# zeromq/libzmq

Hardware: AMD Instinct MI355X
Metric: GiB/s device-resident CURVE encode+decode, 1 KiB-msg batches; msgs/s (higher is better)
Workload: dtype u32; 1 GPU; config2: 65536 x 1024 B frames, 1 CURVE session per GPU, encode+decode round trip; frames_per_gpu=65536, payload_bytes=1024, wire_bytes=1057, sessions=1, parallelism=frame-sharded x1, no collective

## Files before the change

### libzmq_amd/csrc/curve_device.hpp

```cpp
#pragma once

#include <hip/hip_runtime.h>
#include <stdint.h>

namespace zmqg {

__device__ __forceinline__ uint32_t rotl32(uint32_t x, uint32_t n)
{
    return __builtin_rotateleft32(x, n);
}

#define ZMQG_QR(a, b, c, d)        \
    b ^= rotl32(a + d, 7);         \
    c ^= rotl32(b + a, 9);         \
    d ^= rotl32(c + b, 13);        \
    a ^= rotl32(d + c, 18);

#define ZMQG_SALSA20_ROUNDS(x)                                   \
    _Pragma("unroll") for (int rr_ = 0; rr_ < 10; ++rr_)         \
    {                                                            \
        ZMQG_QR(x[0], x[4], x[8], x[12]);                        \
        ZMQG_QR(x[5], x[9], x[13], x[1]);                        \
        ZMQG_QR(x[10], x[14], x[2], x[6]);                       \
        ZMQG_QR(x[15], x[3], x[7], x[11]);                       \
// ... 355 lines not shown
        a = poly32_add(h, c[8], c[9], c[10], c[11], 1u);
    } else {
        a = poly32_add(h, c[0], c[1], c[2], c[3], 1u);
        a = poly32_mul_add<true>(a, k, c[4], c[5], c[6], c[7], 1u);
        a = poly32_mul_add<true>(a, k, c[8], c[9], c[10], c[11], 1u);
    }
    a = poly32_mul_add<true>(a, k, c[12], c[13], c[14], c[15], 1u);
    h = poly32_mul_add<false>(a, k, 0u, 0u, 0u, 0u, 0u);
}

__device__ __forceinline__ PolyKey32 poly32_key_from_fe(const uint32_t r[5])
{
    return poly32_key(r[0] | (r[1] << 26), (r[1] >> 6) | (r[2] << 20), (r[2] >> 12) | (r[3] << 14),
                      (r[3] >> 18) | (r[4] << 8));
}

__device__ __forceinline__ Poly32 fe_to_poly32(fe x)
{
    uint32_t c;
    c = x.l[0] >> 26;
    x.l[0] &= M26;
    x.l[1] += c;
    c = x.l[1] >> 26;
    x.l[1] &= M26;
    x.l[2] += c;
    c = x.l[2] >> 26;
    x.l[2] &= M26;
    x.l[3] += c;
    c = x.l[3] >> 26;
    x.l[3] &= M26;
    x.l[4] += c;
    Poly32 h;
    h.h0 = x.l[0] | (x.l[1] << 26);
    h.h1 = (x.l[1] >> 6) | (x.l[2] << 20);
    h.h2 = (x.l[2] >> 12) | (x.l[3] << 14);
    h.h3 = (x.l[3] >> 18) | (x.l[4] << 8);
    h.h4 = x.l[4] >> 24;
    return h;
}

__device__ __forceinline__ fe poly32_to_fe(const Poly32 &h)
{
    fe x;
    x.l[0] = h.h0 & M26;
    x.l[1] = ((h.h0 >> 26) | (h.h1 << 6)) & M26;
    x.l[2] = ((h.h1 >> 20) | (h.h2 << 12)) & M26;
    x.l[3] = ((h.h2 >> 14) | (h.h3 << 18)) & M26;
    x.l[4] = (h.h3 >> 8) | (h.h4 << 24);
    return x;
}

__device__ __forceinline__ void poly32_finish(const Poly32 &h, const uint32_t s[4], uint32_t tag[4])
{
    unsigned c;
    const uint32_t g0 = __builtin_addc(h.h0, 5u, 0u, &c);
    const uint32_t g1 = __builtin_addc(h.h1, 0u, c, &c);
    const uint32_t g2 = __builtin_addc(h.h2, 0u, c, &c);
    const uint32_t g3 = __builtin_addc(h.h3, 0u, c, &c);
    const uint32_t g4 = h.h4 + c;
    const uint32_t m = 0u - (g4 >> 2);
    const uint32_t f0 = (g0 & m) | (h.h0 & ~m), f1 = (g1 & m) | (h.h1 & ~m), f2 = (g2 & m) | (h.h2 & ~m),
                   f3 = (g3 & m) | (h.h3 & ~m);
    tag[0] = __builtin_addc(f0, s[0], 0u, &c);
    tag[1] = __builtin_addc(f1, s[1], c, &c);
    tag[2] = __builtin_addc(f2, s[2], c, &c);
    tag[3] = __builtin_addc(f3, s[3], c, &c);
}

__device__ __forceinline__ uint32_t bswap32(uint32_t x)
{
    return __builtin_bswap32(x);
}

__device__ __forceinline__ void mask_tail(uint32_t w[16], int nv)
{
#pragma unroll
    for (int i = 0; i < 16; ++i) {
        const int b = nv - 4 * i;
        const uint32_t m = b >= 4 ? 0xffffffffu : (b <= 0 ? 0u : ((1u << (8 * b)) - 1u));
        w[i] &= m;
    }
}

__device__ __forceinline__ void load_window(const uint8_t *p, int nv, uint32_t w[16])
{
    const uint32_t sh = (uint32_t) ((uintptr_t) p & 3);
    const uint32_t *q = (const uint32_t *) (p - sh);
    uint32_t d[17];
    if (nv >= 64) {
#pragma unroll
        for (int i = 0; i < 16; ++i)
            d[i] = q[i];
        d[16] = sh ? q[16] : 0u;
    } else {
        const int nd = (int) ((sh + (uint32_t) nv + 3) >> 2);
#pragma unroll
        for (int i = 0; i < 17; ++i)
            d[i] = i < nd ? q[i] : 0u;
    }
#pragma unroll
    for (int i = 0; i < 16; ++i)
        w[i] = __builtin_amdgcn_alignbyte(d[i + 1], d[i], sh);
    if (nv < 64)
        mask_tail(w, nv);
}

__device__ __forceinline__ void store_window(uint8_t *p, int nv, const uint32_t w[16])
{
    const uintptr_t a = (uintptr_t) p;
    const uint32_t sh = (uint32_t) (a & 3);
    if (sh == 0 && nv >= 64) {
        typedef unsigned int u32x4_ __attribute__((ext_vector_type(4)));
        typedef __attribute__((address_space(1))) u32x4_ __attribute__((aligned(4))) GU4a4_;
#pragma unroll
        for (int i = 0; i < 4; ++i)
            *(GU4a4_ *) (a + 16u * i) = (u32x4_){w[4 * i], w[4 * i + 1], w[4 * i + 2], w[4 * i + 3]};
        return;
    }
    const uint32_t s = (4u - sh) & 3u;
    (void) a;
    uint32_t e[16];
#pragma unroll
    for (int k = 0; k < 15; ++k)
        e[k] = __builtin_amdgcn_alignbyte(w[k + 1], w[k], s);
    e[15] = __builtin_amdgcn_alignbyte(0u, w[15], s);
    const int lead = (int) s < nv ? (int) s : nv;
#pragma unroll
    for (int b = 0; b < 3; ++b)
        if (b < lead)
            p[b] = (uint8_t) (w[0] >> (8 * b));
    if (nv <= (int) s)
        return;
    const int rem = nv - (int) s;
    const int nd = rem >> 2;
    uint32_t *q = (uint32_t *) (p + s);
#pragma unroll
    for (int k = 0; k < 16; ++k)
        if (k < nd)
            q[k] = e[k];
    const int tb = rem & 3;
    if (tb) {
        uint32_t t = 0;
#pragma unroll
        for (int k = 0; k < 16; ++k)
            if (k == nd)
                t = e[k];
        uint8_t *pt = (uint8_t *) (q + nd);
#pragma unroll
        for (int b = 0; b < 3; ++b)
            if (b < tb)
                pt[b] = (uint8_t) (t >> (8 * b));
    }
}

template <int NV>
__device__ __forceinline__ void store_bytes_c(uint8_t *p, const uint32_t w[16])
{
    static_assert(NV % 4 == 0 && NV >= 8 && NV <= 64, "whole dwords, at most one window");
    typedef __attribute__((address_space(1))) uint8_t GU8_;
    typedef __attribute__((address_space(1))) uint16_t GU16_;
    typedef __attribute__((address_space(1))) uint32_t GU32_;
    typedef unsigned int u32x2_ __attribute__((ext_vector_type(2)));
    typedef unsigned int u32x3_ __attribute__((ext_vector_type(3)));
    typedef __attribute__((address_space(1))) u32x2_ __attribute__((aligned(4))) GU2a4_;
    typedef __attribute__((address_space(1))) u32x3_ __attribute__((aligned(4))) GU3a4_;
    typedef unsigned int u32x4_ __attribute__((ext_vector_type(4)));
    typedef __attribute__((address_space(1))) u32x4_ __attribute__((aligned(4))) GU4a4_;
    const uint64_t a = (uint64_t) (uintptr_t) p;
    const uint32_t sh = (uint32_t) a & 3u, s = (4u - sh) & 3u;
    constexpr int ND = NV / 4;
    uint32_t e[ND];
#pragma unroll
    for (int k = 0; k < ND; ++k)
        e[k] = __builtin_amdgcn_alignbyte(k + 1 < 16 ? w[k + 1] : 0u, w[k], s);
    if (s & 1u)
        *(GU8_ *) (uintptr_t) a = (uint8_t) w[0];
    if (s & 2u)
        *(GU16_ *) (uintptr_t) (a + (s & 1u)) = (uint16_t) (w[0] >> (8u * (s & 1u)));
    const uint64_t q = a + s;
    constexpr int NU = ND - 1;
#pragma unroll
    for (int g = 0; g + 4 <= NU; g += 4)
        *(GU4a4_ *) (uintptr_t) (q + 4u * g) = (u32x4_){e[g], e[g + 1], e[g + 2], e[g + 3]};
    constexpr int G4 = NU / 4 * 4;
    if (NU - G4 == 3)
        *(GU3a4_ *) (uintptr_t) (q + 4u * G4) = (u32x3_){e[G4], e[G4 + 1], e[G4 + 2]};
    else if (NU - G4 == 2)
        *(GU2a4_ *) (uintptr_t) (q + 4u * G4) = (u32x2_){e[G4], e[G4 + 1]};
    else if (NU - G4 == 1)
        *(GU32_ *) (uintptr_t) (q + 4u * G4) = e[G4];
    if (s == 0u)
        *(GU32_ *) (uintptr_t) (q + 4u * NU) = e[NU];
    const uint64_t t = q + 4u * NU;
    if (sh & 2u)
        *(GU16_ *) (uintptr_t) t = (uint16_t) e[NU];
    if (sh & 1u)
        *(GU8_ *) (uintptr_t) (t + (sh & 2u)) = (uint8_t) (e[NU] >> (8u * (sh & 2u)));
}

template <int NV>
__device__ __forceinline__ void load_bytes_c(const uint8_t *p, uint32_t w[NV / 4])
{
    static_assert(NV % 16 == 0 && NV >= 16 && NV <= 48, "whole granules");
    typedef __attribute__((address_space(1))) const uint32_t GCU32_;
    typedef unsigned int u32x4_ __attribute__((ext_vector_type(4)));
    typedef __attribute__((address_space(1))) const u32x4_ __attribute__((aligned(4))) GCU4a4_;
    const uint64_t a = (uint64_t) (uintptr_t) p;
    const uint32_t sh = (uint32_t) a & 3u;
    const uint64_t q = a - sh;
    constexpr int ND = NV / 4;
    uint32_t d[ND + 1];
#pragma unroll
    for (int g = 0; g < ND / 4; ++g) {
        const u32x4_ t = *(GCU4a4_ *) (uintptr_t) (q + 16u * g);
        d[4 * g] = t.x;
        d[4 * g + 1] = t.y;
        d[4 * g + 2] = t.z;
        d[4 * g + 3] = t.w;
    }
    d[ND] = sh ? *(GCU32_ *) (uintptr_t) (q + 4u * ND) : 0u;
#pragma unroll
    for (int k = 0; k < ND; ++k)
        w[k] = __builtin_amdgcn_alignbyte(d[k + 1], d[k], sh);
}

__device__ __forceinline__ void store_tail(uint64_t a, uint32_t nb, const uint32_t o[17])
{
    typedef __attribute__((address_space(1))) uint8_t GU8_;
    typedef __attribute__((address_space(1))) uint16_t GU16_;
    typedef __attribute__((address_space(1))) uint32_t GU32_;
    typedef unsigned int u32x4_ __attribute__((ext_vector_type(4)));
    typedef __attribute__((address_space(1))) u32x4_ __attribute__((aligned(4))) GU4a4_;
    const uint32_t nw = nb >> 2, ng = nw >> 2;
#pragma unroll
    for (uint32_t g = 0; g < 4; ++g)
        if (g < ng)
            *(GU4a4_ *) (uintptr_t) (a + 16u * g) = (u32x4_){o[4 * g], o[4 * g + 1], o[4 * g + 2], o[4 * g + 3]};
    uint32_t r[4];
#pragma unroll
    for (uint32_t k = 0; k < 4; ++k) {
        uint32_t v = 0;
#pragma unroll
        for (uint32_t g = 0; g < 5; ++g)
            if (g == ng && 4 * g + k < 17)
                v = o[4 * g + k];
        r[k] = v;
    }
    const uint64_t b = a + 16u * ng;
    const uint32_t nr = nw - 4u * ng;
#pragma unroll
    for (uint32_t k = 0; k < 3; ++k)
        if (k < nr)
            *(GU32_ *) (uintptr_t) (b + 4u * k) = r[k];
    uint32_t last = r[0];
#pragma unroll
    for (uint32_t k = 1; k < 4; ++k)
        if (k == nr)
            last = r[k];
    const uint32_t tb = nb & 3u;
    const uint64_t c = b + 4u * nr;
    if (tb & 2u)
        *(GU16_ *) (uintptr_t) c = (uint16_t) last;
    if (tb & 1u)
        *(GU8_ *) (uintptr_t) (c + (tb & 2u)) = (uint8_t) (last >> (8u * (tb & 2u)));
}

__device__ __forceinline__ void zero_bytes(uint8_t *p, uint32_t len)
{
    const uint32_t head = (uint32_t) ((16u - ((uintptr_t) p & 15u)) & 15u);
    const uint32_t h = head < len ? head : len;
    for (uint32_t b = 0; b < h; ++b)
        p[b] = 0;
    uint32_t k = h;
    typedef unsigned int z4 __attribute__((ext_vector_type(4)));
    for (; k + 16u <= len; k += 16u)
        *(z4 *) (p + k) = (z4){0u, 0u, 0u, 0u};
    for (; k < len; ++k)
        p[k] = 0;
}

typedef unsigned int u32x4 __attribute__((ext_vector_type(4)));
typedef __attribute__((address_space(1))) uint8_t GU8;
typedef __attribute__((address_space(1))) const u32x4 GCU4;
typedef __attribute__((address_space(1))) u32x4 GU4;
typedef __attribute__((address_space(1))) uint32_t GU32;

template <int N>
__device__ __forceinline__ void select_shift(const uint32_t *v, uint32_t ws, uint32_t *out)
{
    const uint32_t m1 = 0u - (ws & 1u), m2 = 0u - ((ws >> 1) & 1u);
    uint32_t a[N + 2];
#pragma unroll
    for (int i = 0; i < N + 2; ++i)
        a[i] = (v[i + 1] & m1) | (v[i] & ~m1);
#pragma unroll
    for (int i = 0; i < N; ++i)
        out[i] = (a[i + 2] & m2) | (a[i] & ~m2);
}

struct StreamReader {
    const GCU4 *g;
    uint32_t off;
    uint32_t end;
// ... 163 lines not shown
```

### libzmq_amd/csrc/curve_frames.hpp

```cpp
#pragma once

#include "../../include/zmqg_curve.h"
#include "curve_device.hpp"
#include "curve_lbrec.hpp"
#include <type_traits>

namespace zmqg {

constexpr uint32_t kFramesBS = 256, kFramesWaves = kFramesBS / 64;

__device__ __forceinline__ void seq_store4(uint64_t a, uint32_t x, uint32_t y, uint32_t z, uint32_t w)
{
    typedef unsigned int v4_ __attribute__((ext_vector_type(4)));
    typedef __attribute__((address_space(1))) v4_ __attribute__((aligned(4))) G4_;
    *(G4_ *) (uintptr_t) a = (v4_){x, y, z, w};
}

#ifndef ZMQG_SEQ_STAMPS
#define ZMQG_SEQ_STAMPS 0
#endif

#if ZMQG_SEQ_STAMPS
#define SEQ_STAMP(slot)                                                                            \
    do {                                                                                           \
// ... 308 lines not shown
        __hip_atomic_store(&zs->done, 0u, __ATOMIC_RELAXED, __HIP_MEMORY_SCOPE_AGENT);
        __hip_atomic_store(&zs->ticket, 0u, __ATOMIC_RELAXED, __HIP_MEMORY_SCOPE_AGENT);
        __hip_atomic_store(&zs->epoch, c.epoch + 1u, __ATOMIC_RELAXED, __HIP_MEMORY_SCOPE_AGENT);
        if (!DEC && ctl.nonce_ctr)
            __hip_atomic_store(ctl.nonce_ctr, c.nbase + n, __ATOMIC_RELAXED, __HIP_MEMORY_SCOPE_AGENT);
    }
}

constexpr uint32_t kLaneFillMax = 4608;

__device__ __forceinline__ unsigned long long lookback_excl(uint32_t t, uint32_t epoch,
                                                            const unsigned long long *lb_flag,
                                                            const unsigned long long *lb_agg,
                                                            const unsigned long long *lb_inc)
{
    __shared__ uint32_t sh_stop[kFramesWaves];
    __shared__ unsigned long long sh_v[kFramesWaves];
    const uint32_t tid = threadIdx.x, lane = tid & 63u, wv = tid >> 6;
    unsigned long long P = 0;
    for (int base = (int) t; base > 0; base -= (int) kFramesBS) {
        const int k = base - 1 - (int) tid;
        int state = 2;
        if (k >= 0) {
            unsigned long long f;
            do {
                f = __hip_atomic_load(lb_flag + k, __ATOMIC_RELAXED, __HIP_MEMORY_SCOPE_AGENT);
            } while ((uint32_t) (f >> 2) != epoch || (f & 3ull) == 0);
            state = (int) (f & 3ull);
        }
        unsigned long long v = 0;
        if (k >= 0)
            v = __hip_atomic_load((state == 2 ? lb_inc : lb_agg) + k, __ATOMIC_RELAXED, __HIP_MEMORY_SCOPE_AGENT);
        const unsigned long long m = __ballot(state == 2);
        if (lane == 0)
            sh_stop[wv] = m ? 64u * wv + (uint32_t) __builtin_ctzll(m) : kFramesBS;
        __syncthreads();
        uint32_t stop = kFramesBS;
        for (uint32_t w = 0; w < kFramesWaves; ++w)
            stop = sh_stop[w] < stop ? sh_stop[w] : stop;
        if (tid > stop)
            v = 0;
#pragma unroll
        for (int d = 32; d >= 1; d >>= 1) {
            const unsigned long long o = __shfl_xor(v, d);
            v = o > v ? o : v;
        }
        if (lane == 0)
            sh_v[wv] = v;
        __syncthreads();
        for (uint32_t w = 0; w < kFramesWaves; ++w)
            P = sh_v[w] > P ? sh_v[w] : P;
        __syncthreads();
        if (stop < kFramesBS)
            break;
    }
    return P;
}

__device__ __forceinline__ void lookback_publish(unsigned long long *flag, unsigned long long *val,
                                                 unsigned long long v, uint32_t epoch, uint32_t state)
{
    __hip_atomic_store(val, v, __ATOMIC_RELAXED, __HIP_MEMORY_SCOPE_AGENT);
    asm volatile("s_waitcnt vmcnt(0)" ::: "memory");
    __hip_atomic_store(flag, ((unsigned long long) epoch << 2) | state, __ATOMIC_RELAXED, __HIP_MEMORY_SCOPE_AGENT);
}

__device__ __forceinline__ void fail_unprocessed(int32_t status, uint32_t L_in, uint8_t *dst, uint8_t *flags_out,
                                                 int32_t *status_out, ZState *zs, const FrameCtl &ctl)
{
    *status_out = status;
    *flags_out = 0;
    if (status == ZMQG_ERR_BOUND || L_in < 33u)
        return;
    if (L_in - 33u <= kLaneFillMax || ctl.post == nullptr)
        zero_bytes(dst, L_in - 33u);
    else
        post_append(zs, ctl.post, (uint64_t) (uintptr_t) dst, L_in - 33u, kPostZero, 0);
}

struct NoBigFrames {
    __device__ void operator()(uint32_t, unsigned long long *, uint64_t) const {}
};

#define ZMQG_FRAMES_PARAMS                                                                                    \
    uint32_t n, const uint32_t *__restrict__ sid, const uint64_t *__restrict__ nonce,                             \
        const uint8_t *__restrict__ flags, const uint64_t *__restrict__ in_off, const uint32_t *__restrict__ len, \
        const uint8_t *__restrict__ in, const uint64_t *__restrict__ out_off, uint8_t *__restrict__ out,          \
        const DevSession *__restrict__ sessions, uint32_t max_sessions, uint32_t max_stream,                      \
        uint8_t *__restrict__ flags_out, int32_t *__restrict__ status_out, ReplayOut rp, BigOp big,               \
        ZState *__restrict__ zs, FrameCtl ctl
#define ZMQG_FRAMES_ARGS                                                                                      \
    n, sid, nonce, flags, in_off, len, in, out_off, out, sessions, max_sessions, max_stream, flags_out,           \
        status_out, rp, big, zs, ctl

template <bool DEC, int G, class BigOp>
__device__ __forceinline__ void frames_g_impl(ZMQG_FRAMES_PARAMS)
{
    static_assert(G == 1 || G == 2 || G == 4 || G == 8, "lanes per frame");
    const bool lb = DEC && rp.lb_flag != nullptr;
    unsigned long long clk0 = 0, rclk0 = 0;
    if (rp.clk) {
        clk0 = __builtin_amdgcn_s_memtime();
        rclk0 = __builtin_amdgcn_s_memrealtime();
    }
    __shared__ unsigned long long sh_wmax[kFramesWaves];
    const bool use_ticket = lb && !rp.ordered && !(rp.dbg & 2);
    const CallState cs = call_state_begin<DEC>(zs, ctl, use_ticket);
    const uint32_t epoch = cs.epoch;
    const uint32_t wg = use_ticket ? cs.ticket : blockIdx.x;
    const uint64_t nbase = cs.nbase;
    unsigned long long *const list_ctr = zs->list_ctr + (epoch & 1u);
    if (blockIdx.x == 0 && threadIdx.x == 0)
        zs->list_ctr[(epoch & 1u) ^ 1u] = 0;
    const uint32_t gl = (wg - ctl.split_wg) * kFramesBS + threadIdx.x;
    const uint32_t lane = threadIdx.x & 63u;
    const uint32_t i = ctl.split_n + gl / G, q = gl % G;
    const uint32_t gbase = lane - q;
    const bool valid = i < n;
    const uint32_t ii = valid ? i : n - 1;
    const bool sid_ok = sid[ii] < max_sessions;
    const uint32_t s = sid_ok ? sid[ii] : 0u;
    const DevSession &ses = sessions[s];
    uint32_t key[8];
#pragma unroll
    for (int t = 0; t < 8; ++t)
        key[t] = DEC ? ses.dec_key[t] : ses.enc_key[t];
    const uint8_t *src = in + in_off[ii];
    uint8_t *dst = out + out_off[ii];
    const uint32_t L_in = len[ii];
    const bool over = frame_over<DEC>(ctl, L_in, out_off[ii]);

    uint32_t S = 0, n0 = 0, n1 = 0, hl = 1;
    uint64_t A = 0, B = 0;
    int32_t status = 0;
    uint32_t hw[3] = {0, 0, 0};
    if (!DEC) {
        const uint64_t nc = frame_nonce(nonce, ctl, nbase, ii);
        n0 = bswap32((uint32_t) (nc >> 32));
        n1 = bswap32((uint32_t) nc);
        hl = plaintext_header(flags[ii], ses.downgrade_sub, hw);
        S = sid_ok && !over ? 32u + hl + L_in : 0u;
        A = (uint64_t) (uintptr_t) src - 32u - hl;
        B = (uint64_t) (uintptr_t) dst;
    } else {
        uint32_t h16[16];
        load_window(src, L_in < 16u ? (int) L_in : 16, h16);
        const uint32_t b0 = h16[0] & 0xffu;
        if (L_in <= 1u || L_in <= b0)
            status = ZMQG_ERR_MALFORMED_UNSPECIFIED;
        else if (L_in < 8u || h16[0] != 0x53454d07u || h16[1] != 0x45474153u)
            status = ZMQG_ERR_UNEXPECTED_COMMAND;
        else if (L_in < 33u)
            status = ZMQG_ERR_MALFORMED_MESSAGE;
        if (!sid_ok)
            status = ZMQG_ERR_SESSION;
        if (over)
            status = ZMQG_ERR_BOUND;
        n0 = h16[2];
        n1 = h16[3];
        S = status == 0 ? L_in : 0u;
        A = (uint64_t) (uintptr_t) src;
        B = (uint64_t) (uintptr_t) dst - 33u;
    }
    const bool small = valid && S <= max_stream;
    unsigned long long vn = 0, wexcl = 0, psn = 0, wagg = 0;
    if (DEC) {
        vn = valid && q == 0 && status == 0 ? (((unsigned long long) bswap32(n0) << 32) | bswap32(n1)) : 0ull;
// ... 326 lines not shown
            asm volatile("s_waitcnt vmcnt(0)" ::: "memory");
            zero_bytes(dst, S - 33u);
        }
    }
}

template <bool DEC, int G, class BigOp>
__global__ __launch_bounds__(kFramesBS) void k_frames(ZMQG_FRAMES_PARAMS)
{
    frames_g_impl<DEC, G, BigOp>(ZMQG_FRAMES_ARGS);
}

template <int CTRL, int ROWS>
__device__ __forceinline__ unsigned long long dpp_u64(unsigned long long v)
{
    const uint32_t lo = (uint32_t) __builtin_amdgcn_update_dpp(0, (int) (uint32_t) v, CTRL, ROWS, 0xf, true);
    const uint32_t hi = (uint32_t) __builtin_amdgcn_update_dpp(0, (int) (uint32_t) (v >> 32), CTRL, ROWS, 0xf, true);
    return ((unsigned long long) hi << 32) | lo;
}
__device__ __forceinline__ unsigned long long max_u64(unsigned long long a, unsigned long long b)
{
    return a > b ? a : b;
}
__device__ __forceinline__ unsigned long long wave_scan_max_u64(unsigned long long v)
{
    v = max_u64(v, dpp_u64<0x111, 0xf>(v));
    v = max_u64(v, dpp_u64<0x112, 0xf>(v));
    v = max_u64(v, dpp_u64<0x114, 0xf>(v));
    v = max_u64(v, dpp_u64<0x118, 0xf>(v));
    v = max_u64(v, dpp_u64<0x142, 0xa>(v));
    v = max_u64(v, dpp_u64<0x143, 0xc>(v));
    return v;
}
__device__ __forceinline__ unsigned long long wave_prev_u64(unsigned long long v)
{
    return dpp_u64<0x138, 0xf>(v);
}
__device__ __forceinline__ unsigned long long wave_max_u64(unsigned long long v)
{
    v = max_u64(v, dpp_u64<0x111, 0xf>(v));
    v = max_u64(v, dpp_u64<0x112, 0xf>(v));
    v = max_u64(v, dpp_u64<0x114, 0xf>(v));
    v = max_u64(v, dpp_u64<0x118, 0xf>(v));
    unsigned long long m = 0;
#pragma unroll
    for (int r = 15; r < 64; r += 16) {
        const unsigned long long x = ((unsigned long long) (uint32_t) __builtin_amdgcn_readlane((int) (uint32_t) (v >> 32), r) << 32) |
                                     (uint32_t) __builtin_amdgcn_readlane((int) (uint32_t) v, r);
        m = max_u64(m, x);
    }
    return m;
}
__device__ __forceinline__ uint32_t wave_max_u32(uint32_t v)
{
    auto mx = [](uint32_t a, uint32_t b) { return a > b ? a : b; };
    v = mx(v, (uint32_t) __builtin_amdgcn_update_dpp(0, (int) v, 0x111, 0xf, 0xf, true));
    v = mx(v, (uint32_t) __builtin_amdgcn_update_dpp(0, (int) v, 0x112, 0xf, 0xf, true));
    v = mx(v, (uint32_t) __builtin_amdgcn_update_dpp(0, (int) v, 0x114, 0xf, 0xf, true));
    v = mx(v, (uint32_t) __builtin_amdgcn_update_dpp(0, (int) v, 0x118, 0xf, 0xf, true));
    return mx(mx((uint32_t) __builtin_amdgcn_readlane((int) v, 15), (uint32_t) __builtin_amdgcn_readlane((int) v, 31)),
              mx((uint32_t) __builtin_amdgcn_readlane((int) v, 47), (uint32_t) __builtin_amdgcn_readlane((int) v, 63)));
}

constexpr uint32_t kStIn = 80;
typedef u32x4 u32x4_u1 __attribute__((aligned(1)));
typedef __attribute__((address_space(3))) void StLdsVoid;

__device__ __forceinline__ void lds_dma16(uint64_t gaddr, uint32_t lds_base)
{
    unsigned keep;
    asm volatile("s_mov_b32 %0, m0\n\ts_mov_b32 m0, %2\n\ts_nop 0\n\tglobal_load_lds_dwordx4 %1, off\n\ts_mov_b32 m0, %0"
                 : "=&s"(keep)
                 : "v"(gaddr), "s"(lds_base)
                 : "memory");
}

__device__ __forceinline__ uint64_t shfl_u64(uint64_t v, uint32_t src)
{
    const uint32_t lo = (uint32_t) __shfl((int) (uint32_t) v, (int) src);
    const uint32_t hi = (uint32_t) __shfl((int) (uint32_t) (v >> 32), (int) src);
    return ((uint64_t) hi << 32) | lo;
}

template <bool DEC, class BigOp, bool SO = false>
__device__ __forceinline__ void frames_seq_impl(ZMQG_FRAMES_PARAMS)
{
    const bool lb = DEC && rp.lb_flag != nullptr;
    const bool use_rec = lb && rp.ordered && rp.lb_rec != nullptr && gridDim.x <= kFramesBS &&
                         ctl.split_wg == 0;
    const uint32_t nlim = ctl.split_wg ? ctl.split_n : n;
    SEQ_STAMP(0u);
    __shared__ unsigned long long sh_wmax[kFramesWaves];
    __shared__ CallState sh_cs;
    const bool use_ticket = lb && !rp.ordered;
    const uint32_t lane = threadIdx.x & 63u;

    uint32_t i = 0, ii = 0, s = 0, L_in = 0;
    bool valid = false, sid_ok = false, over = false;
    const uint8_t *src = nullptr;
    uint8_t *dst = nullptr;
    uint32_t key[8];
    uint32_t S = 0, n0 = 0, n1 = 0, hl = 1;
    uint64_t A = 0, B = 0;
    int32_t status = 0;
    uint32_t hw[3] = {0, 0, 0};
    uint32_t x0[16];
    auto fetch = [&](uint32_t wgv) {
        i = wgv * kFramesBS + threadIdx.x;
        valid = i < nlim;
        ii = valid ? i : nlim - 1;
        sid_ok = sid[ii] < max_sessions;
        s = sid_ok ? sid[ii] : 0u;
        const DevSession &ses = sessions[s];
#pragma unroll
        for (int t = 0; t < 8; ++t)
            key[t] = DEC ? ses.dec_key[t] : ses.enc_key[t];
        src = in + in_off[ii];
        dst = out + out_off[ii];
        L_in = len[ii];
        over = frame_over<DEC>(ctl, L_in, out_off[ii]);
        if (!DEC) {
            hl = plaintext_header(flags[ii], ses.downgrade_sub, hw);
            S = sid_ok && !over ? 32u + hl + L_in : 0u;
            A = (uint64_t) (uintptr_t) src - 32u - hl;
            B = (uint64_t) (uintptr_t) dst;
            if (L_in >= 32u) {
                load_bytes_c<32>(src, x0);
#pragma unroll
                for (int k = 8; k < 16; ++k)
                    x0[k] = 0;
            } else {
                load_window(src, (int) L_in, x0);
            }
        } else {
            A = (uint64_t) (uintptr_t) src;
            uint32_t d[17];
            frame_load_raw(A, 0, L_in, d);
#pragma unroll
            for (int k = 0; k < 16; ++k)
                x0[k] = __builtin_amdgcn_alignbyte(d[k + 1], d[k], (uint32_t) A & 3u);
            B = (uint64_t) (uintptr_t) dst - 33u;
        }
    };
    CallState c0{};
    if (threadIdx.x == 0) {
        c0.epoch = __hip_atomic_load(&zs->epoch, __ATOMIC_RELAXED, __HIP_MEMORY_SCOPE_AGENT);
        c0.ticket = use_ticket ? atomicAdd(&zs->ticket, 1u) : 0u;
        c0.nbase = DEC ? 0ull : nonce_base(ctl);
    }
    if (!use_ticket)
        fetch(blockIdx.x);
    if (threadIdx.x == 0)
        sh_cs = c0;
    __syncthreads();
    const CallState cs = sh_cs;
    const uint32_t epoch = cs.epoch;
    const uint32_t wg = use_ticket ? cs.ticket : blockIdx.x;
    if (use_ticket)
        fetch(wg);
    const uint64_t nbase = cs.nbase;
    unsigned long long *const list_ctr = zs->list_ctr + (epoch & 1u);
    if (blockIdx.x == 0 && threadIdx.x == 0)
        zs->list_ctr[(epoch & 1u) ^ 1u] = 0;

    if (!DEC) {
        const uint64_t nc = frame_nonce(nonce, ctl, nbase, ii);
        n0 = bswap32((uint32_t) (nc >> 32));
        n1 = bswap32((uint32_t) nc);
    } else {
        if (L_in < 64u)
            mask_tail(x0, (int) L_in);
        const uint32_t b0 = x0[0] & 0xffu;
        if (L_in <= 1u || L_in <= b0)
            status = ZMQG_ERR_MALFORMED_UNSPECIFIED;
        else if (L_in < 8u || x0[0] != 0x53454d07u || x0[1] != 0x45474153u)
            status = ZMQG_ERR_UNEXPECTED_COMMAND;
        else if (L_in < 33u)
            status = ZMQG_ERR_MALFORMED_MESSAGE;
        if (!sid_ok)
            status = ZMQG_ERR_SESSION;
        if (over)
            status = ZMQG_ERR_BOUND;
        n0 = x0[2];
        n1 = x0[3];
        S = status == 0 ? L_in : 0u;
    }
    const bool small = valid && S <= max_stream;
    unsigned long long vn = 0, wexcl = 0, psn = 0, wagg = 0;
    if (DEC) {
        vn = valid && status == 0 ? (((unsigned long long) bswap32(n0) << 32) | bswap32(n1)) : 0ull;
        psn = rp.peer[s];
        if (valid && !lb) {
            rp.vout[i] = vn;
            rp.psnap[i] = psn;
            if (rp.iota)
                rp.iota[i] = i;
        }
        if (lb) {
            const unsigned long long sc = wave_scan_max_u64(vn);
            const unsigned long long up = wave_prev_u64(sc);
            if (lane == 63)
                sh_wmax[threadIdx.x >> 6] = sc;
            __syncthreads();
            const uint32_t wv = threadIdx.x >> 6;
            for (uint32_t k = 0; k < kFramesWaves; ++k) {
                if (k < wv)
                    wexcl = sh_wmax[k] > wexcl ? sh_wmax[k] : wexcl;
                wagg = sh_wmax[k] > wagg ? sh_wmax[k] : wagg;
            }
            if (lane > 0)
                wexcl = up > wexcl ? up : wexcl;
            if (threadIdx.x == 0) {
                if (use_rec) {
                    __hip_atomic_store(rp.lb_rec + 2u * wg, lbrec_pack(epoch, (uint32_t) wagg), __ATOMIC_RELAXED,
                                       __HIP_MEMORY_SCOPE_AGENT);
                    __hip_atomic_store(rp.lb_rec + 2u * wg + 1u, lbrec_pack(epoch, (uint32_t) (wagg >> 32)),
                                       __ATOMIC_RELAXED, __HIP_MEMORY_SCOPE_AGENT);
                } else {
                    lookback_publish(rp.lb_flag + wg, rp.lb_agg + wg, wagg, epoch, 1);
                }
            }
        }
    }
    const bool is_big = valid && !small && S > 0;
    if (!small)
        S = 0;
    const uint32_t nw = (S + 63u) >> 6;
    const uint32_t steps = __builtin_amdgcn_readfirstlane(wave_max_u32(nw));
    __shared__ __attribute__((aligned(16))) uint8_t sq_lds[kFramesWaves * 2 * 64 * kStIn];
    uint8_t *const sq_w = sq_lds + (threadIdx.x >> 6) * 2 * 64 * kStIn;
    const uint32_t sq_off = __builtin_amdgcn_readfirstlane((uint32_t) (uintptr_t) (StLdsVoid *) sq_w);
    const uint32_t sq_va = (uint32_t) A & 15u;
    uint64_t sq_la[5];
    uint32_t sq_rel[5], sq_lim[5];
    {
        const uint64_t Ab = A - sq_va;
        const uint32_t lm = S ? sq_va + S : 0u;
#pragma unroll
        for (uint32_t j = 0; j < 5; ++j) {
            const uint32_t idx = 64u * j + lane, f = idx / 5u, k = idx - 5u * f;
            sq_rel[j] = 16u * k;
            sq_la[j] = shfl_u64(Ab, f) + sq_rel[j];
            sq_lim[j] = (uint32_t) __shfl((int) lm, (int) f);
            const int fva = __shfl((int) sq_va, (int) f);
            if (k == 4u && fva == 0)
                sq_lim[j] = 0;
        }
    }
    auto sq_dma = [&](uint32_t t) {
        const uint32_t b = __builtin_amdgcn_readfirstlane(sq_off + (t & 1u) * 64u * kStIn);
#pragma unroll
        for (uint32_t j = 0; j < 5; ++j)
            if (64u * t + sq_rel[j] < sq_lim[j])
                lds_dma16(sq_la[j] + 64ull * t, b + 1024u * j);
    };
    const uint32_t min_nw = __builtin_amdgcn_readfirstlane(~wave_max_u32(~nw));
    uint64_t sq_m[5];
#pragma unroll
    for (uint32_t j = 0; j < 5; ++j)
        sq_m[j] = __builtin_amdgcn_ballot_w64(sq_lim[j] != 0u);
    auto sq_dma_uni = [&](uint32_t t) {
        const uint32_t b = __builtin_amdgcn_readfirstlane(sq_off + (t & 1u) * 64u * kStIn);
        uint64_t a[5];
#pragma unroll
        for (uint32_t j = 0; j < 5; ++j)
            a[j] = sq_la[j] + 64ull * t;
        unsigned keep;
        uint64_t ex;
        asm volatile("s_mov_b32 %0, m0\n\t"
                     "s_mov_b64 %1, exec\n\t"
                     "s_mov_b32 m0, %7\n\t"
                     "s_mov_b64 exec, %8\n\t"
                     "global_load_lds_dwordx4 %2, off\n\t"
                     "s_add_u32 m0, m0, 0x400\n\t"
                     "s_mov_b64 exec, %9\n\t"
                     "global_load_lds_dwordx4 %3, off\n\t"
                     "s_add_u32 m0, m0, 0x400\n\t"
                     "s_mov_b64 exec, %10\n\t"
                     "global_load_lds_dwordx4 %4, off\n\t"
                     "s_add_u32 m0, m0, 0x400\n\t"
                     "s_mov_b64 exec, %11\n\t"
                     "global_load_lds_dwordx4 %5, off\n\t"
                     "s_add_u32 m0, m0, 0x400\n\t"
                     "s_mov_b64 exec, %12\n\t"
                     "global_load_lds_dwordx4 %6, off\n\t"
                     "s_mov_b64 exec, %1\n\t"
                     "s_mov_b32 m0, %0"
                     : "=&s"(keep), "=&s"(ex)
                     : "v"(a[0]), "v"(a[1]), "v"(a[2]), "v"(a[3]), "v"(a[4]), "s"(b), "s"(sq_m[0]), "s"(sq_m[1]),
                       "s"(sq_m[2]), "s"(sq_m[3]), "s"(sq_m[4])
                     : "memory", "scc");
    };
    if (steps > 1u)
        sq_dma(1u);

    const bool al64 = DEC && __builtin_amdgcn_ballot_w64(((uint32_t) (uintptr_t) dst & 63u) != 0u) == 0;
    uint32_t yp[16];
    bool cs_pend = false;
    constexpr uint32_t kStgPlane = 64u * 16u + 16u;
    __shared__ __attribute__((aligned(16))) uint8_t sq_stg[SO ? kFramesWaves * 4 * kStgPlane : 16];
    uint8_t *const stg = sq_stg + (SO ? (threadIdx.x >> 6) * 4u * kStgPlane : 0u);
    auto stg_put = [&](uint32_t k) { return stg + kStgPlane * k + 16u * lane; };
    auto stg_get = [&](uint32_t j) { return stg + kStgPlane * (lane & 3u) + 16u * (16u * j + (lane >> 2)); };
    uint64_t cs_dst[4];
    uint32_t cs_nw[4];
    const bool coop = SO && (DEC ? al64 : true);
    if (coop) {
        const uint64_t cbase = DEC ? (uint64_t) (uintptr_t) dst : B - (((uint32_t) B & 3u) ? ((uint32_t) B & 3u) : 4u);
#pragma unroll
        for (uint32_t j = 0; j < 4; ++j) {
            const uint32_t f = 16u * j + (lane >> 2);
            cs_dst[j] = shfl_u64(cbase, f) + 16u * (lane & 3u);
            cs_nw[j] = (uint32_t) __shfl((int) nw, (int) f);
        }
    }
    uint32_t ct0[8];

    SEQ_STAMP(1u);
    PolyKey32 pk;
    Poly32 h = {0, 0, 0, 0, 0};
    uint32_t spad[4], wtag[4] = {0, 0, 0, 0}, fl = 0;
    uint32_t cp[16];
    uint32_t cp_j0 = 2, cp_len = 0;
    uint32_t ycarry;
    {
        uint32_t ks[16];
        salsa20_block(ks, key, n0, n1, 0, 0);
        pk = poly32_key(ks[0], ks[1], ks[2], ks[3]);
#pragma unroll
        for (int k = 0; k < 4; ++k)
            spad[k] = ks[4 + k];
        uint32_t x[16];
        if (DEC) {
#pragma unroll
            for (int k = 0; k < 16; ++k)
                x[k] = x0[k];
#pragma unroll
            for (int k = 0; k < 4; ++k)
                wtag[k] = x[4 + k];
        } else {
            uint32_t pt[8];
            switch (hl) {
            case 1: shift_in<1>(x0, pt); break;
            case 2: shift_in<2>(x0, pt); break;
            case 8: shift_in<8>(x0, pt); break;
            default: shift_in<11>(x0, pt); break;
            }
            pt[0] |= hw[0];
            pt[1] |= hw[1];
            pt[2] |= hw[2];
#pragma unroll
            for (int k = 0; k < 8; ++k) {
                x[k] = 0;
                x[8 + k] = pt[k];
            }
        }
        uint32_t y[16];
#pragma unroll
        for (int k = 0; k < 16; ++k)
            y[k] = x[k] ^ ks[k];
        if (!DEC && S < 64u)
            mask_tail(y, (int) S);
#pragma unroll
        for (int k = 0; k < 16; ++k)
            cp[k] = DEC ? x[k] : y[k];
        cp_len = (S < 64u ? S : 64u) - 32u;
        ycarry = y[15];
#pragma unroll
        for (int k = 0; k < 16; ++k)
            yp[k] = y[k];
        if (nw > 0) {
            if (DEC) {
                fl = y[8] & 3u;
                uint32_t pay[16];
#pragma unroll
                for (int k = 0; k < 7; ++k)
                    pay[k] = __builtin_amdgcn_alignbyte(y[9 + k], y[8 + k], 1);
                pay[7] = __builtin_amdgcn_alignbyte(0u, y[15], 1);
#pragma unroll
                for (int k = 8; k < 16; ++k)
                    pay[k] = 0;
                if (!al64 || nw == 1u)
                    store_window(dst, (int) (S < 64u ? S : 64u) - 33, pay);
            } else {
#pragma unroll
                for (int k = 0; k < 8; ++k)
                    ct0[k] = y[8 + k];
                if (S < 64u) {
                    uint32_t o[16];
                    o[0] = 0x53454d07u;
                    o[1] = 0x45474153u;
                    o[2] = n0;
                    o[3] = n1;
#pragma unroll
                    for (int k = 4; k < 16; ++k)
                        o[k] = 0;
                    store_bytes_c<16>(dst, o);
                    uint32_t ct[16];
#pragma unroll
                    for (int k = 0; k < 16; ++k)
                        ct[k] = k < 8 ? y[8 + k] : 0u;
                    store_window(dst + 32, (int) S - 32, ct);
                }
            }
        }
    }
    SEQ_STAMP(2u);
    call_state_count(zs);

    auto step = [&](auto uni, uint32_t t) {
// ... 161 lines not shown
        }
        ycarry = y[15];
        if (t < 8u)
            SEQ_STAMP(36u + t);
    };
    if (steps > 1u) {
#pragma unroll 1
        for (uint32_t t = 1; t < steps; ++t) {
            if (t + 2u < min_nw)
                step(std::true_type{}, t);
            else
                step(std::false_type{}, t);
        }
    }
    SEQ_STAMP(60u);
    unsigned long long rl[4] = {0, 0, 0, 0}, rh[4] = {0, 0, 0, 0};
    if (use_rec) {
#pragma unroll
        for (uint32_t q = 0; q < 4; ++q) {
            const int k = (int) wg - 1 - (int) (lane + 64u * q);
            const unsigned long long *const r = rp.lb_rec + 2u * (uint32_t) (k >= 0 ? k : 0);
            rl[q] = __hip_atomic_load(r, __ATOMIC_RELAXED, __HIP_MEMORY_SCOPE_AGENT);
            rh[q] = __hip_atomic_load(r + 1, __ATOMIC_RELAXED, __HIP_MEMORY_SCOPE_AGENT);
        }
        asm volatile("" : "+v"(h.h0), "+v"(h.h1), "+v"(h.h2), "+v"(h.h3), "+v"(h.h4)::"memory");
    }
    if (steps > 0 && nw == steps)
        poly32_window(h, pk, cp, cp_j0, cp_len);
    uint32_t tag[4];
    poly32_finish(h, spad, tag);

    unsigned long long excl = 0;
    if (use_rec) {
        unsigned long long P = 0;
#pragma unroll
        for (uint32_t q = 0; q < 4; ++q) {
            const int k = (int) wg - 1 - (int) (lane + 64u * q);
            if (k >= 0) {
                const unsigned long long *const r = rp.lb_rec + 2u * (uint32_t) k;
                while (!lbrec_valid(rl[q], epoch)) {
                    __builtin_amdgcn_s_sleep(1);
                    rl[q] = __hip_atomic_load(r, __ATOMIC_RELAXED, __HIP_MEMORY_SCOPE_AGENT);
                }
                while (!lbrec_valid(rh[q], epoch)) {
                    __builtin_amdgcn_s_sleep(1);
                    rh[q] = __hip_atomic_load(r + 1, __ATOMIC_RELAXED, __HIP_MEMORY_SCOPE_AGENT);
                }
                P = max_u64(P, lbrec_value(rl[q], rh[q]));
            }
        }
        P = wave_max_u64(P);
        if (threadIdx.x == 0 && wg + 1 == gridDim.x) {
            const unsigned long long inc = P > wagg ? P : wagg;
            *rp.peer = inc > psn ? inc : psn;
            if (rp.smax)
                *rp.smax = inc;
        }
        excl = P > wexcl ? P : wexcl;
        if (excl < psn)
            excl = psn;
    } else if (lb) {
        const unsigned long long P = lookback_excl(wg, epoch, rp.lb_flag, rp.lb_agg, rp.lb_inc);
        if (threadIdx.x == 0) {
            const unsigned long long inc = P > wagg ? P : wagg;
            if (gridDim.x > kFramesBS)
                lookback_publish(rp.lb_flag + wg, rp.lb_inc + wg, inc, epoch, 2);
            if (wg + 1 == gridDim.x) {
                *rp.peer = inc > psn ? inc : psn;
                if (rp.smax)
                    *rp.smax = inc;
            }
        }
        excl = P > wexcl ? P : wexcl;
        if (excl < psn)
            excl = psn;
    }
    if (is_big && !ctl.no_body) {
        if (lb) {
            rp.excl[i] = excl;
            rp.psnap[i] = psn;
        }
        big(i, list_ctr, nbase);
    }
    call_state_end<DEC>(zs, ctl, cs, n);
    frame_result_copy<DEC>(big);
    SEQ_STAMP(61u);
#if ZMQG_SEQ_STAMPS
    if (rp.clk && (threadIdx.x & 63u) == 0)
        rp.clk[64ull * (blockIdx.x * kFramesWaves + (threadIdx.x >> 6)) + 62u] =
            ((unsigned long long) __builtin_amdgcn_s_getreg((31 << 11) | 20) << 32) |
            __builtin_amdgcn_s_getreg((31 << 11) | 4);
#endif
    if (!DEC && valid && ctl.enc_status)
        ctl.enc_status[i] = !sid_ok ? ZMQG_ERR_SESSION : over ? ZMQG_ERR_BOUND : 0;
    if (!valid || !small)
        return;
    if (S == 0) {
        if (DEC)
            fail_unprocessed(status, L_in, dst, flags_out + i, status_out + i, zs, ctl);
        return;
    }
    if (!DEC) {
        if (S >= 64u) {
            const uint32_t o[16] = {0x53454d07u, 0x45474153u, n0,     n1,     tag[0], tag[1], tag[2], tag[3],
                                    ct0[0],      ct0[1],      ct0[2], ct0[3], ct0[4], ct0[5], ct0[6], ct0[7]};
            store_bytes_c<64>(dst, o);
        } else {
            const uint32_t o[16] = {tag[0], tag[1], tag[2], tag[3]};
            store_bytes_c<16>(dst + 16, o);
        }
    } else {
        if (lb && !(vn > excl))
            status = ZMQG_ERR_INVALID_SEQUENCE;
        else if ((tag[0] ^ wtag[0]) | (tag[1] ^ wtag[1]) | (tag[2] ^ wtag[2]) | (tag[3] ^ wtag[3]))
            status = ZMQG_ERR_CRYPTOGRAPHIC;
        status_out[i] = status;
        flags_out[i] = status == 0 ? (uint8_t) (fl | frame_zbits<DEC>(big, i)) : 0;
        if (status != 0) {
            asm volatile("s_waitcnt vmcnt(0)" ::: "memory");
            zero_bytes(dst, S - 33u);
        }
    }
}

template <bool DEC, class BigOp, bool SO = false>
__global__ __launch_bounds__(kFramesBS) void k_frames_seq(ZMQG_FRAMES_PARAMS)
{
    frames_seq_impl<DEC, BigOp, SO>(ZMQG_FRAMES_ARGS);
}

template <bool DEC, int GT, class BigOp>
__global__ __launch_bounds__(kFramesBS) void k_frames_split(ZMQG_FRAMES_PARAMS)
{
    if (blockIdx.x < ctl.split_wg)
        frames_seq_impl<DEC, BigOp>(ZMQG_FRAMES_ARGS);
    else
        frames_g_impl<DEC, GT, BigOp>(ZMQG_FRAMES_ARGS);
}

}
```

Before: 653.1 GiB/s.

## Overlap frame prologue loads with first Salsa20 block and drop the startup barrier

Restructures the per-frame kernel prologue. Kernarg lines are prefetched, and every metadata load (sid, offsets, len, flags, nonce, epoch, nonce counter, peer snapshot) is issued together. The raw payload window is loaded early and only realigned after the first Salsa20 block, so memory latency overlaps the keystream computation. In the non-relay path, thread 0 no longer broadcasts the call state through shared memory behind a barrier; each lane reads epoch and nonce base itself, with a barrier placed after the keystream block instead. The cost is more live registers and redundant per-lane atomic loads, and the list_ctr reset moves to the end of the kernel, which could change ordering semantics.

After: 661.1 GiB/s (median of 6 runs). 1.2% higher.

```diff
diff --git a/libzmq_amd/csrc/curve_device.hpp b/libzmq_amd/csrc/curve_device.hpp
--- a/libzmq_amd/csrc/curve_device.hpp
+++ b/libzmq_amd/csrc/curve_device.hpp
@@ -461,6 +461,15 @@
     }
 }
 
+template <int ND>
+__device__ __forceinline__ void load_window_raw(const uint32_t *q, uint32_t sh, int nv, uint32_t d[ND])
+{
+    const int nd = (int) ((sh + (uint32_t) nv + 3) >> 2);
+#pragma unroll
+    for (int i = 0; i < ND; ++i)
+        d[i] = i < nd ? q[i] : 0u;
+}
+
 __device__ __forceinline__ void load_window(const uint8_t *p, int nv, uint32_t w[16])
 {
     const uint32_t sh = (uint32_t) ((uintptr_t) p & 3);
@@ -472,10 +481,7 @@
             d[i] = q[i];
         d[16] = sh ? q[16] : 0u;
     } else {
-        const int nd = (int) ((sh + (uint32_t) nv + 3) >> 2);
-#pragma unroll
-        for (int i = 0; i < 17; ++i)
-            d[i] = i < nd ? q[i] : 0u;
+        load_window_raw<17>(q, sh, nv, d);
     }
 #pragma unroll
     for (int i = 0; i < 16; ++i)
@@ -578,7 +584,7 @@
 }
 
 template <int NV>
-__device__ __forceinline__ void load_bytes_c(const uint8_t *p, uint32_t w[NV / 4])
+__device__ __forceinline__ void load_bytes_raw(const uint8_t *p, uint32_t d[NV / 4 + 1])
 {
     static_assert(NV % 16 == 0 && NV >= 16 && NV <= 48, "whole granules");
     typedef __attribute__((address_space(1))) const uint32_t GCU32_;
@@ -588,7 +594,6 @@
     const uint32_t sh = (uint32_t) a & 3u;
     const uint64_t q = a - sh;
     constexpr int ND = NV / 4;
-    uint32_t d[ND + 1];
 #pragma unroll
     for (int g = 0; g < ND / 4; ++g) {
         const u32x4_ t = *(GCU4a4_ *) (uintptr_t) (q + 16u * g);
@@ -598,6 +603,15 @@
         d[4 * g + 3] = t.w;
     }
     d[ND] = sh ? *(GCU32_ *) (uintptr_t) (q + 4u * ND) : 0u;
+}
+
+template <int NV>
+__device__ __forceinline__ void load_bytes_c(const uint8_t *p, uint32_t w[NV / 4])
+{
+    constexpr int ND = NV / 4;
+    uint32_t d[ND + 1];
+    load_bytes_raw<NV>(p, d);
+    const uint32_t sh = (uint32_t) (uintptr_t) p & 3u;
 #pragma unroll
     for (int k = 0; k < ND; ++k)
         w[k] = __builtin_amdgcn_alignbyte(d[k + 1], d[k], sh);
diff --git a/libzmq_amd/csrc/curve_frames.hpp b/libzmq_amd/csrc/curve_frames.hpp
--- a/libzmq_amd/csrc/curve_frames.hpp
+++ b/libzmq_amd/csrc/curve_frames.hpp
@@ -414,7 +414,7 @@
     __device__ void operator()(uint32_t, unsigned long long *, uint64_t) const {}
 };
 
-#define ZMQG_FRAMES_PARAMS                                                                                    \
+#define ZMQG_FRAMES_PARAMS                                                                                   \
     uint32_t n, const uint32_t *__restrict__ sid, const uint64_t *__restrict__ nonce,                             \
         const uint8_t *__restrict__ flags, const uint64_t *__restrict__ in_off, const uint32_t *__restrict__ len, \
         const uint8_t *__restrict__ in, const uint64_t *__restrict__ out_off, uint8_t *__restrict__ out,          \
@@ -907,17 +907,58 @@
     return ((uint64_t) hi << 32) | lo;
 }
 
+template <class BigOp>
+struct FramesKernarg {
+    uint32_t n;
+    const void *sid, *nonce, *flags, *in_off, *len, *in, *out_off, *out, *sessions;
+    uint32_t max_sessions, max_stream;
+    void *flags_out, *status_out;
+    ReplayOut rp;
+    BigOp big;
+    ZState *zs;
+    FrameCtl ctl;
+};
+
+template <size_t BYTES>
+__device__ __forceinline__ void kernarg_touch()
+{
+    typedef __attribute__((address_space(4))) const uint32_t KA32;
+    KA32 *const ka = (KA32 *) __builtin_amdgcn_kernarg_segment_ptr();
+    constexpr int NL = (int) ((BYTES + 8 + 63) / 64);
+    uint32_t t[NL];
+#pragma unroll
+    for (int q = 0; q < NL; ++q)
+        t[q] = ka[16 * q];
+    static_assert(NL >= 1 && NL <= 8, "one statement's operands");
+    auto at = [&](int q) { return t[q < NL ? q : NL - 1]; };
+    asm volatile("" ::"s"(at(0)), "s"(at(1)), "s"(at(2)), "s"(at(3)), "s"(at(4)), "s"(at(5)), "s"(at(6)), "s"(at(7)));
+}
+
 template <bool DEC, class BigOp, bool SO = false>
 __device__ __forceinline__ void frames_seq_impl(ZMQG_FRAMES_PARAMS)
 {
+#if ZMQG_SEQ_STAMPS
+    const unsigned long long clk_entry = __builtin_amdgcn_s_memtime();
+#endif
+    kernarg_touch<sizeof(FramesKernarg<BigOp>)>();
+#if ZMQG_SEQ_STAMPS
+    const unsigned long long clk_args = __builtin_amdgcn_s_memtime();
+#endif
     const bool lb = DEC && rp.lb_flag != nullptr;
     const bool use_rec = lb && rp.ordered && rp.lb_rec != nullptr && gridDim.x <= kFramesBS &&
                          ctl.split_wg == 0;
     const uint32_t nlim = ctl.split_wg ? ctl.split_n : n;
     SEQ_STAMP(0u);
+#if ZMQG_SEQ_STAMPS
+    if (rp.clk && (threadIdx.x & 63u) == 0) {
+        rp.clk[64ull * (blockIdx.x * kFramesWaves + (threadIdx.x >> 6)) + 20u] = clk_entry;
+        rp.clk[64ull * (blockIdx.x * kFramesWaves + (threadIdx.x >> 6)) + 21u] = clk_args;
+    }
+#endif
     __shared__ unsigned long long sh_wmax[kFramesWaves];
     __shared__ CallState sh_cs;
     const bool use_ticket = lb && !rp.ordered;
+    const bool relay = use_ticket || ctl.split_wg != 0;
     const uint32_t lane = threadIdx.x & 63u;
 
     uint32_t i = 0, ii = 0, s = 0, L_in = 0;
@@ -930,71 +971,109 @@
     int32_t status = 0;
     uint32_t hw[3] = {0, 0, 0};
     uint32_t x0[16];
+    uint32_t dr[17], sh0 = 0;
+    uint64_t ncv = 0;
+    unsigned long long psn = 0;
+    uint32_t dg = 0;
+    uint32_t w_epoch = 0;
+    uint64_t w_nbase = 0;
     auto fetch = [&](uint32_t wgv) {
         i = wgv * kFramesBS + threadIdx.x;
         valid = i < nlim;
         ii = valid ? i : nlim - 1;
-        sid_ok = sid[ii] < max_sessions;
-        s = sid_ok ? sid[ii] : 0u;
+        if (!relay) {
+            w_epoch = __hip_atomic_load(&zs->epoch, __ATOMIC_RELAXED, __HIP_MEMORY_SCOPE_AGENT);
+            if (!DEC && ctl.nonce_ctr)
+                w_nbase = __hip_atomic_load(ctl.nonce_ctr, __ATOMIC_RELAXED, __HIP_MEMORY_SCOPE_AGENT);
+        }
+        uint32_t sidv = sid[ii];
+        uint64_t ioff = in_off[ii], ooff = out_off[ii];
+        L_in = len[ii];
+        uint32_t mfl = 0;
+        if (!DEC) {
+            mfl = flags[ii];
+            if (!ctl.nonce_ctr)
+                ncv = nonce[ii];
+        }
+        asm volatile(""
+                     : "+v"(sidv), "+v"(ioff), "+v"(ooff), "+v"(L_in), "+v"(mfl), "+v"(ncv), "+v"(w_epoch),
+                       "+v"(w_nbase)::"memory");
+        sid_ok = sidv < max_sessions;
+        s = sid_ok ? sidv : 0u;
         const DevSession &ses = sessions[s];
 #pragma unroll
         for (int t = 0; t < 8; ++t)
             key[t] = DEC ? ses.dec_key[t] : ses.enc_key[t];
-        src = in + in_off[ii];
-        dst = out + out_off[ii];
-        L_in = len[ii];
-        over = frame_over<DEC>(ctl, L_in, out_off[ii]);
+        src = in + ioff;
+        dst = out + ooff;
+        over = frame_over<DEC>(ctl, L_in, ooff);
         if (!DEC) {
-            hl = plaintext_header(flags[ii], ses.downgrade_sub, hw);
+            dg = ses.downgrade_sub;
+            sh0 = (uint32_t) (uintptr_t) src & 3u;
+            if (L_in >= 32u)
+                load_bytes_raw<32>(src, dr);
+            else
+                load_window_raw<9>((const uint32_t *) (src - sh0), sh0, (int) L_in, dr);
+            asm volatile("" ::: "memory");
+            hl = plaintext_header(mfl, dg, hw);
             S = sid_ok && !over ? 32u + hl + L_in : 0u;
             A = (uint64_t) (uintptr_t) src - 32u - hl;
             B = (uint64_t) (uintptr_t) dst;
-            if (L_in >= 32u) {
-                load_bytes_c<32>(src, x0);
-#pragma unroll
-                for (int k = 8; k < 16; ++k)
-                    x0[k] = 0;
-            } else {
-                load_window(src, (int) L_in, x0);
-            }
         } else {
             A = (uint64_t) (uintptr_t) src;
-            uint32_t d[17];
-            frame_load_raw(A, 0, L_in, d);
-#pragma unroll
-            for (int k = 0; k < 16; ++k)
-                x0[k] = __builtin_amdgcn_alignbyte(d[k + 1], d[k], (uint32_t) A & 3u);
+            sh0 = (uint32_t) A & 3u;
+            frame_load_raw(A, 0, L_in, dr);
+            psn = rp.peer[s];
+            asm volatile("" ::: "memory");
             B = (uint64_t) (uintptr_t) dst - 33u;
         }
     };
     CallState c0{};
-    if (threadIdx.x == 0) {
-        c0.epoch = __hip_atomic_load(&zs->epoch, __ATOMIC_RELAXED, __HIP_MEMORY_SCOPE_AGENT);
-        c0.ticket = use_ticket ? atomicAdd(&zs->ticket, 1u) : 0u;
-        c0.nbase = DEC ? 0ull : nonce_base(ctl);
-    }
-    if (!use_ticket)
+    if (!relay) {
         fetch(blockIdx.x);
-    if (threadIdx.x == 0)
-        sh_cs = c0;
-    __syncthreads();
-    const CallState cs = sh_cs;
+        SEQ_STAMP(22u);
+        uint32_t e = __builtin_amdgcn_readfirstlane(w_epoch);
+        uint32_t b0 = __builtin_amdgcn_readfirstlane((uint32_t) w_nbase);
+        uint32_t b1 = __builtin_amdgcn_readfirstlane((uint32_t) (w_nbase >> 32));
+        asm volatile("" : "+s"(e), "+s"(b0), "+s"(b1));
+        c0.epoch = e;
+        c0.nbase = ((uint64_t) b1 << 32) | b0;
+    } else {
+        if (threadIdx.x == 0) {
+            c0.epoch = __hip_atomic_load(&zs->epoch, __ATOMIC_RELAXED, __HIP_MEMORY_SCOPE_AGENT);
+            c0.ticket = use_ticket ? atomicAdd(&zs->ticket, 1u) : 0u;
+            c0.nbase = DEC ? 0ull : nonce_base(ctl);
+        }
+        if (!use_ticket)
+            fetch(blockIdx.x);
+        if (threadIdx.x == 0)
+            sh_cs = c0;
+        __syncthreads();
+        c0 = sh_cs;
+        if (use_ticket)
+            fetch(c0.ticket);
+    }
+    const CallState cs = c0;
     const uint32_t epoch = cs.epoch;
     const uint32_t wg = use_ticket ? cs.ticket : blockIdx.x;
-    if (use_ticket)
-        fetch(wg);
     const uint64_t nbase = cs.nbase;
     unsigned long long *const list_ctr = zs->list_ctr + (epoch & 1u);
-    if (blockIdx.x == 0 && threadIdx.x == 0)
-        zs->list_ctr[(epoch & 1u) ^ 1u] = 0;
 
     if (!DEC) {
-        const uint64_t nc = frame_nonce(nonce, ctl, nbase, ii);
+        const uint64_t nc = ctl.nonce_ctr ? nbase + ii : ncv;
         n0 = bswap32((uint32_t) (nc >> 32));
         n1 = bswap32((uint32_t) nc);
     } else {
-        if (L_in < 64u)
-            mask_tail(x0, (int) L_in);
+#pragma unroll
+        for (int k = 0; k < 4; ++k)
+            x0[k] = __builtin_amdgcn_alignbyte(dr[k + 1], dr[k], sh0);
+        if (L_in < 16u) {
+            uint32_t t[16] = {x0[0], x0[1], x0[2], x0[3]};
+            mask_tail(t, (int) L_in);
+#pragma unroll
+            for (int k = 0; k < 4; ++k)
+                x0[k] = t[k];
+        }
         const uint32_t b0 = x0[0] & 0xffu;
         if (L_in <= 1u || L_in <= b0)
             status = ZMQG_ERR_MALFORMED_UNSPECIFIED;
@@ -1010,40 +1089,43 @@
         n1 = x0[3];
         S = status == 0 ? L_in : 0u;
     }
+#if ZMQG_SEQ_STAMPS
+    asm volatile("" : "+v"(S), "+v"(n0), "+v"(n1));
+#endif
+    SEQ_STAMP(23u);
     const bool small = valid && S <= max_stream;
-    unsigned long long vn = 0, wexcl = 0, psn = 0, wagg = 0;
+    unsigned long long vn = 0, wexcl = 0, wagg = 0;
     if (DEC) {
         vn = valid && status == 0 ? (((unsigned long long) bswap32(n0) << 32) | bswap32(n1)) : 0ull;
-        psn = rp.peer[s];
         if (valid && !lb) {
             rp.vout[i] = vn;
             rp.psnap[i] = psn;
             if (rp.iota)
                 rp.iota[i] = i;
         }
-        if (lb) {
-            const unsigned long long sc = wave_scan_max_u64(vn);
-            const unsigned long long up = wave_prev_u64(sc);
-            if (lane == 63)
-                sh_wmax[threadIdx.x >> 6] = sc;
-            __syncthreads();
-            const uint32_t wv = threadIdx.x >> 6;
-            for (uint32_t k = 0; k < kFramesWaves; ++k) {
-                if (k < wv)
-                    wexcl = sh_wmax[k] > wexcl ? sh_wmax[k] : wexcl;
-                wagg = sh_wmax[k] > wagg ? sh_wmax[k] : wagg;
-            }
-            if (lane > 0)
-                wexcl = up > wexcl ? up : wexcl;
-            if (threadIdx.x == 0) {
-                if (use_rec) {
-                    __hip_atomic_store(rp.lb_rec + 2u * wg, lbrec_pack(epoch, (uint32_t) wagg), __ATOMIC_RELAXED,
-                                       __HIP_MEMORY_SCOPE_AGENT);
-                    __hip_atomic_store(rp.lb_rec + 2u * wg + 1u, lbrec_pack(epoch, (uint32_t) (wagg >> 32)),
-                                       __ATOMIC_RELAXED, __HIP_MEMORY_SCOPE_AGENT);
-                } else {
-                    lookback_publish(rp.lb_flag + wg, rp.lb_agg + wg, wagg, epoch, 1);
-                }
+    }
+    if (lb) {
+        const unsigned long long sc = wave_scan_max_u64(vn);
+        const unsigned long long up = wave_prev_u64(sc);
+        if (lane == 63)
+            sh_wmax[threadIdx.x >> 6] = sc;
+        __syncthreads();
+        const uint32_t wv = threadIdx.x >> 6;
+        for (uint32_t k = 0; k < kFramesWaves; ++k) {
+            if (k < wv)
+                wexcl = sh_wmax[k] > wexcl ? sh_wmax[k] : wexcl;
+            wagg = sh_wmax[k] > wagg ? sh_wmax[k] : wagg;
+        }
+        if (lane > 0)
+            wexcl = up > wexcl ? up : wexcl;
+        if (threadIdx.x == 0) {
+            if (use_rec) {
+                __hip_atomic_store(rp.lb_rec + 2u * wg, lbrec_pack(epoch, (uint32_t) wagg), __ATOMIC_RELAXED,
+                                   __HIP_MEMORY_SCOPE_AGENT);
+                __hip_atomic_store(rp.lb_rec + 2u * wg + 1u, lbrec_pack(epoch, (uint32_t) (wagg >> 32)),
+                                   __ATOMIC_RELAXED, __HIP_MEMORY_SCOPE_AGENT);
+            } else {
+                lookback_publish(rp.lb_flag + wg, rp.lb_agg + wg, wagg, epoch, 1);
             }
         }
     }
@@ -1116,6 +1198,10 @@
                        "s"(sq_m[2]), "s"(sq_m[3]), "s"(sq_m[4])
                      : "memory", "scc");
     };
+#pragma unroll
+    for (int t = 0; t < 8; ++t)
+        asm volatile("" : "+v"(key[t]));
+    asm volatile("" : "+v"(n0), "+v"(n1));
     if (steps > 1u)
         sq_dma(1u);
 
@@ -1151,6 +1237,34 @@
     {
         uint32_t ks[16];
         salsa20_block(ks, key, n0, n1, 0, 0);
+#pragma unroll
+        for (int k = 0; k < 16; ++k)
+            asm volatile("" : "+v"(ks[k]));
+        SEQ_STAMP(24u);
+        if (!relay)
+            __syncthreads();
+#pragma unroll
+        for (int k = DEC ? 5 : 0; k < (DEC ? 17 : 9); ++k)
+            asm volatile("" : "+v"(dr[k]));
+        if (!DEC)
+            asm volatile("" : "+v"(dg));
+        if (DEC) {
+#pragma unroll
+            for (int k = 4; k < 16; ++k)
+                x0[k] = __builtin_amdgcn_alignbyte(dr[k + 1], dr[k], sh0);
+            if (L_in < 64u)
+                mask_tail(x0, (int) L_in);
+        } else {
+#pragma unroll
+            for (int k = 0; k < 8; ++k)
+                x0[k] = __builtin_amdgcn_alignbyte(dr[k + 1], dr[k], sh0);
+#pragma unroll
+            for (int k = 8; k < 16; ++k)
+                x0[k] = 0;
+            if (L_in < 32u)
+                mask_tail(x0, (int) L_in);
+        }
+        SEQ_STAMP(63u);
         pk = poly32_key(ks[0], ks[1], ks[2], ks[3]);
 #pragma unroll
         for (int k = 0; k < 4; ++k)
@@ -1478,6 +1592,8 @@
         }
         big(i, list_ctr, nbase);
     }
+    if (blockIdx.x == 0 && threadIdx.x == 0)
+        zs->list_ctr[(epoch & 1u) ^ 1u] = 0;
     call_state_end<DEC>(zs, ctl, cs, n);
     frame_result_copy<DEC>(big);
     SEQ_STAMP(61u);
```
